# schusterbenjamin/Vision-Language-Pretraining-for-Bone-Tumor-Detection

Hardware: AMD Instinct MI355X
Metric: image-text pairs/sec (fwd+bwd) at bs=256/GPU, 1/2/4/8 MI355X (higher is better)
Workload: dtype bf16; 1 GPU; ResNet34+TinyBERT CLIP pretrain step (fwd+bwd+global-batch InfoNCE+AdamW); global_batch=256, per_gpu_batch=256, image_size=512, seq_len=40, parallelism=dp1

## Files before the change

include/vlp_hip.h:

```cpp
#ifndef VLP_HIP_H
#define VLP_HIP_H
#include <stdint.h>
#ifdef __cplusplus
extern "C" {
#endif

int vlp_abi_version(void);
int vlp_mfma_peak_probe(int blocks, int iters, float* out, void* stream);
int vlp_trace_marker(int end, void* stream);

int vlp_conv_fwd(int dtype, const void* x, const void* wp, void* y, int N, int H, int W, int C,
                 int Co, int KH, int KW, int S, int P, const float* in_scale,
                 const float* in_shift, double* stat_sum, double* stat_sumsq, int stat_rep,
                 void* stream);
int vlp_conv_fwd_act_ok(int dtype, int N, int H, int W, int C, int Co, int KH, int KW, int S, int P);
int vlp_conv_fwd_act(int dtype, const void* x, const void* wp, void* y, void* x_act, int N, int H, int W,
                     int C, int Co, int KH, int KW, int S, int P, const float* in_scale,
                     const float* in_shift, double* stat_sum, double* stat_sumsq, int stat_rep,
                     void* stream);
int vlp_conv_dgrad(int dtype, const void* dy, const void* wt, void* dx, int N, int H, int W, int C,
                   int Co, int KH, int KW, int S, int P, const void* addend, const void* y_bn,
                   const float* bn_scale, const float* bn_shift, const float* bn_mean,
                   const float* bn_invstd, double* stat1, double* stat2, int stat_rep,
                   void* stream);
int vlp_conv_dgrad_relu(int dtype, const void* dy, const void* wt, void* g, int N, int H, int W,
                        int C, int Co, int KH, int KW, int S, int P, const void* addend,
                        const void* relu_out, const uint8_t* relu_mask, const void* y,
                        const float* mean, const float* invstd, double* stat1, double* stat2,
                        int stat_rep, void* stream);
int vlp_conv_dgrad_act_ok(int dtype, int N, int H, int W, int C, int Co, int KH, int KW, int S, int P);
int vlp_conv_dgrad_bn_act(int dtype, const void* g_in, const void* y_in, const float* in_coef, void* dy_out,
                          const void* wt, void* dx, int N, int H, int W, int C, int Co, int KH, int KW,
                          int S, int P, const void* y_bn, const float* bn_scale, const float* bn_shift,
                          const float* bn_mean, const float* bn_invstd, double* stat1, double* stat2,
// ... 201 lines not shown
```

vision-language-pretraining-for-bone-tumor-detection_amd/csrc/bn_ops.hip:

```cpp
#include "common.h"

namespace vlp {

constexpr int kEwThreads = 256;

__device__ __forceinline__ uint8_t relu_bits8(const uint4& u) {
  const unsigned w[4] = {u.x, u.y, u.z, u.w};
  unsigned m = 0;
#pragma unroll
  for (int q = 0; q < 4; ++q) {
    const unsigned lo = w[q] & 0xffffu, hi = w[q] >> 16;
    m |= (unsigned)((lo & 0x8000u) == 0 && lo != 0) << (2 * q);
    m |= (unsigned)((hi & 0x8000u) == 0 && hi != 0) << (2 * q + 1);
  }
  return (uint8_t)m;
}

static inline int ew_blocks(size_t work, int per_block = kEwThreads, int cap = 8192) {
  size_t b = (work + per_block - 1) / per_block;
  if (b > (size_t)cap) b = cap;
  if (b < 1) b = 1;
  return (int)b;
}

__global__ void bn_finalize_kernel(int C, double count, const double* __restrict__ sum,
                                   const double* __restrict__ sumsq, const float* __restrict__ gamma,
                                   const float* __restrict__ beta, float eps, float momentum,
                                   float* running_mean, float* running_var, float* scale,
                                   float* shift, float* mean_out, float* invstd_out) {
  int c = blockIdx.x * blockDim.x + threadIdx.x;
  if (c >= C) return;
// ... 136 lines not shown
  const int c0 = (int)(tid % (unsigned)cpr) * E;
  float a[E], b[E], c[E], d[E];
#pragma unroll
  for (int j = 0; j < E; ++j) {
    a[j] = sc[c0 + j]; b[j] = sh[c0 + j];
    c[j] = scd ? scd[c0 + j] : 1.f;
    d[j] = scd ? shd[c0 + j] : 0.f;
    b[j] += d[j];
  }
  auto one = [&](unsigned i, const uint4& yv, const uint4& iv) __attribute__((always_inline)) {
    float u[E], v[E];
    Chunk<T>::unpack(yv, u);
    if constexpr (HAS_IDT) {
      Chunk<T>::unpack(iv, v);
#pragma unroll
      for (int j = 0; j < E; ++j) u[j] = fmaxf(fmaf(u[j], a[j], fmaf(v[j], c[j], b[j])), 0.f);
    } else {
#pragma unroll
      for (int j = 0; j < E; ++j) u[j] = fmaxf(fmaf(u[j], a[j], b[j]), 0.f);
    }
    const uint4 pk = Chunk<T>::pack(u);
    ew_st16<U, NT>(out + (size_t)i * E, pk);
    if constexpr (E == 8) {
      if (rmask) rmask[i] = relu_bits8(pk);
    }
  };
  unsigned i = tid;
  if constexpr (U > 1) {
    for (; i + (U - 1) * stride < nchunks; i += U * stride) {
      uint4 yv[U], iv[U];
#pragma unroll
// ... 45 lines not shown
      const unsigned i = i0 + 256u * k;
      if (i < nchunks) {
        yv[k] = NTL ? ntl16(y + (size_t)i * 8) : ldg16(y + (size_t)i * 8);
        if constexpr (HAS_IDT) iv[k] = NTL ? ntl16(idt + (size_t)i * 8) : ldg16(idt + (size_t)i * 8);
      }
    }
#pragma unroll
    for (int k = 0; k < U; ++k) {
      const unsigned i = i0 + 256u * k;
      if (i >= nchunks) continue;
      float u[8], v[8];
      Chunk<bf16>::unpack(yv[k], u);
      if constexpr (HAS_IDT) {
        Chunk<bf16>::unpack(iv[k], v);
#pragma unroll
        for (int j = 0; j < 8; ++j) u[j] = fmaxf(fmaf(u[j], a[j], fmaf(v[j], c[j], b[j])), 0.f);
      } else {
#pragma unroll
        for (int j = 0; j < 8; ++j) u[j] = fmaxf(fmaf(u[j], a[j], b[j]), 0.f);
      }
      const uint4 pk = Chunk<bf16>::pack(u);
      ew_st16<1, true>(out + (size_t)i * 8, pk);
      if (rmask) rmask[i] = relu_bits8(pk);
    }
  }
}

template <typename T>
__global__ void __launch_bounds__(256)
bn_bwd_reduce_kernel(int M, int C, const T* __restrict__ dout, const float* __restrict__ dbc,
                     int HW, const T* __restrict__ mask, const T* __restrict__ ya,
// ... 927 lines not shown
```

vision-language-pretraining-for-bone-tumor-detection_amd/csrc/common.h:

```cpp
#pragma once
#include <hip/hip_runtime.h>
#include <stdint.h>

namespace vlp {

typedef __bf16 bf16;
typedef float v4f __attribute__((ext_vector_type(4)));
typedef __bf16 v4bf __attribute__((ext_vector_type(4)));
typedef __bf16 v8bf __attribute__((ext_vector_type(8)));

enum { VLP_F32 = 0, VLP_BF16 = 1 };

template <typename T> struct Elem;
template <> struct Elem<bf16> {
  static constexpr int EPC = 8;
  static constexpr int BK = 64;
};
template <> struct Elem<float> {
  static constexpr int EPC = 4;
  static constexpr int BK = 32;
};

__device__ __forceinline__ float to_f(float x) { return x; }
__device__ __forceinline__ float to_f(bf16 x) { return (float)x; }
// ... 75 lines not shown
  return (t + ((n - t) >> f.s1)) >> f.s2;
}

__device__ __forceinline__ void bn_bwd_coef(float gamma, float istd, float mean, double sum_g, double sum_gx,
                                            float inv_count, float& k, float& b, float& c) {
  k = __fmul_rn(gamma, istd);
  const float mg = __fmul_rn((float)sum_g, inv_count), mgx = __fmul_rn((float)sum_gx, inv_count);
  const float t = __fmul_rn(__fmul_rn(k, istd), mgx);
  b = -t;
  c = __fadd_rn(-__fmul_rn(k, mg), __fmul_rn(t, mean));
}
__device__ __forceinline__ float bn_bwd_dy(float k, float b, float c, float g, float y) {
  return __fmaf_rn(k, g, __fmaf_rn(b, y, c));
}

__device__ __forceinline__ float warp_sum(float v) {
#pragma unroll
  for (int o = 32; o > 0; o >>= 1) v += __shfl_xor(v, o, 64);
  return v;
}
__device__ __forceinline__ float warp_max(float v) {
#pragma unroll
  for (int o = 32; o > 0; o >>= 1) v = fmaxf(v, __shfl_xor(v, o, 64));
  return v;
}

__device__ __forceinline__ float hash_uniform(uint64_t seed, uint64_t idx) {
  uint64_t z = seed + 0x9E3779B97F4A7C15ull * (idx + 1);
  z = (z ^ (z >> 30)) * 0xBF58476D1CE4E5B9ull;
  z = (z ^ (z >> 27)) * 0x94D049BB133111EBull;
// ... 11 lines not shown
```

vision-language-pretraining-for-bone-tumor-detection_amd/csrc/conv_ops.hip:

```cpp
#include "gemm.h"
#include "stem_geom.h"

namespace vlp {

struct ConvGeom {
  int N, H, W, C, Co, KH, KW, S, P, Ho, Wo;
  int M;
  int K;
  FastDiv fd_howo, fd_wo, fd_hw, fd_w, fd_c, fd_co, fd_kw;
};

static ConvGeom make_geom(int N, int H, int W, int C, int Co, int KH, int KW, int S, int P) {
  ConvGeom g;
  g.N = N; g.H = H; g.W = W; g.C = C; g.Co = Co; g.KH = KH; g.KW = KW; g.S = S; g.P = P;
  g.Ho = (H + 2 * P - KH) / S + 1;
  g.Wo = (W + 2 * P - KW) / S + 1;
  g.M = 0; g.K = 0;
  g.fd_howo = make_fastdiv(g.Ho * g.Wo);
  g.fd_wo = make_fastdiv(g.Wo);
  g.fd_hw = make_fastdiv(H * W);
  g.fd_w = make_fastdiv(W);
  g.fd_c = make_fastdiv(C);
  g.fd_co = make_fastdiv(Co);
  g.fd_kw = make_fastdiv(KW);
// ... 1128 lines not shown
constexpr int kRcRing = 5;
constexpr int kRcRingOff = kRcWeights;
constexpr int kRcAux = 0;
constexpr int kRcTail = kRcWeights + kRcRing * kRcSlot;
constexpr int kRcXtab = kRcTail + 2048;
constexpr int kRcLds = kRcXtab + 768;
static_assert(kRcLds <= 160 * 1024, "rows kernel LDS map");

#ifndef VLP_ACT_NT
#define VLP_ACT_NT 0
#endif
struct RowsXIn {
  const float* t0; const float* t1;
  const bf16* y;
  bf16* out;
};
template <class EP, int XF = 0>
__global__ void __launch_bounds__(512)
conv3x3_c64_rows_kernel(int N, int H, const bf16* __restrict__ x, const bf16* __restrict__ w, int flip,
                        EP ep, int M, RowsXIn xin) {
  constexpr int S = RowTrait<EP>::value ? 2 : 4;
  static_assert(XF != 1 || !RowTrait<EP>::value, "forward input transform with the direct epilogue only");
  static_assert(XF != 2 || RowTrait<EP>::value, "backward input transform with a row-chunk epilogue only");
  extern __shared__ __attribute__((aligned(16))) char smem[];
  char* wlds = smem;
  char* ring = smem + kRcRingOff;
  char* aux = smem + kRcAux;
  float* red = reinterpret_cast<float*>(RowTrait<EP>::value ? aux + 16384 : smem + kRcTail);
  const int tid = threadIdx.x, lane = tid & 63;
  const int wv = __builtin_amdgcn_readfirstlane((int)(tid >> 6));
  const int pq = wv & 3, ch = wv >> 2;
  const rsrc_t rx = buf_rsrc(x, (unsigned)((size_t)N * H * kRcW * 64 * 2));
  const rsrc_t rw = buf_rsrc(w, 64 * 576 * 2);
  const rsrc_t rz = null_rsrc(zero_page());

  for (int j = wv; j < 72; j += 8) {
    const int b = j >> 3, q = (j & 7) * 64 + lane;
// ... 46 lines not shown
    __syncthreads();
    v4f* rp = reinterpret_cast<v4f*>(red + tid * 16);
    rp[0] = rp[1] = rp[2] = rp[3] = v4f{0.f, 0.f, 0.f, 0.f};
  }
  constexpr int NCF = CoefTrait<EP>::value;
  float* cfl = reinterpret_cast<float*>(smem + kRcTail);
  if constexpr (NCF > 0) {
    for (int q = tid; q < NCF * 64; q += 512) cfl[q] = ep.coef(q >> 6)[q & 63];
    __syncthreads();
  }
  float* xtab = reinterpret_cast<float*>(smem + kRcXtab);
  if constexpr (XF == 1) {
    if (tid < 128) xtab[tid] = tid < 64 ? xin.t0[tid] : xin.t1[tid - 64];
    __syncthreads();
  }
  if constexpr (XF == 2) {
    if (tid < 192) xtab[tid] = xin.t0[tid];
    __syncthreads();
  }
  char* ybuf = aux + 16384 + 32768;
  static_assert(16384 + 32768 + kRcW * 128 <= kRcWeights, "y row buffer fits the filter area");
  const rsrc_t ry = XF == 2 ? buf_rsrc(xin.y, (unsigned)((size_t)N * H * kRcW * 64 * 2)) : rz;
  auto yload = [&](int n, int r) __attribute__((always_inline)) {
    const bool live = (unsigned)r < (unsigned)H;
    const rsrc_t rr = live ? ry : rz;
    const unsigned base = live ? (unsigned)(((size_t)n * H + r) * kRcW * 128) : 0u;
    int sd = lane;
    asm volatile("" : "+v"(sd));
#pragma unroll
    for (int jj = 0; jj < 2; ++jj) {
      const int j = wv * 2 + jj;
      int px, c;
      piece_src(j, sd, px, c);
      dma16(rr, base + (unsigned)(px * 128 + c * 16), ybuf + j * 1024);
    }
  };
  auto xrow = [&](int n, int r) __attribute__((always_inline)) {
// ... 5 lines not shown
      const int j = wv * 2 + jj, q = j * 64 + sd;
      int px, cc;
      piece_src(j, sd, px, cc);
      uint4* p = reinterpret_cast<uint4*>(piece_lds(slot, j) + sd * 16);
      float f[8];
      Chunk<bf16>::unpack(*p, f);
      if constexpr (XF == 2) {
        float yy[8];
        Chunk<bf16>::unpack(*reinterpret_cast<const uint4*>(ybuf + q * 16), yy);
#pragma unroll
        for (int j = 0; j < 8; ++j)
          f[j] = bn_bwd_dy(xtab[cc * 8 + j], xtab[64 + cc * 8 + j], xtab[128 + cc * 8 + j], f[j], yy[j]);
      } else {
        const v4f s0 = *reinterpret_cast<const v4f*>(xtab + cc * 8), s1 = *reinterpret_cast<const v4f*>(xtab + cc * 8 + 4);
        const v4f h0 = *reinterpret_cast<const v4f*>(xtab + 64 + cc * 8), h1 = *reinterpret_cast<const v4f*>(xtab + 68 + cc * 8);
#pragma unroll
        for (int j = 0; j < 4; ++j) {
          f[j] = fmaxf(fmaf(f[j], s0[j], h0[j]), 0.f);
          f[4 + j] = fmaxf(fmaf(f[4 + j], s1[j], h1[j]), 0.f);
        }
      }
      const uint4 v = Chunk<bf16>::pack(f);
      *p = v;
#if VLP_ACT_NT
      typedef unsigned v4u_nt __attribute__((ext_vector_type(4)));
      __builtin_nontemporal_store(v4u_nt{v.x, v.y, v.z, v.w},
                                  reinterpret_cast<v4u_nt*>(xin.out + (((size_t)n * H + r) * kRcW + px) * 64 + cc * 8));
#else
      stg16(xin.out + (((size_t)n * H + r) * kRcW + px) * 64 + cc * 8, v);
#endif
    }
  };

  for (int n = blockIdx.x; n < N; n += gridDim.x) {
    wait_vmcnt<0>();
    __syncthreads();
    if constexpr (XF == 2) {
      fetch(n, -1); fetch(n, 0); yload(n, 0);
    } else {
      fetch(n, -1); fetch(n, 0); fetch(n, 1); fetch(n, 2);
    }
    for (int i = 0; i < H; ++i) {
      if constexpr (XF == 2) {
        if (i == 0) {
          wait_vmcnt<0>();
          xrow(n, 0);
          yload(n, 1);
          fetch(n, 1);
          fetch(n, 2);
          wait_vmcnt<2>();
          xrow(n, 1);
        } else {
          wait_vmcnt<2 + S>();
          if (i + 1 < H) xrow(n, i + 1);
        }
        asm volatile("s_waitcnt lgkmcnt(0)" ::: "memory");
      } else {
        if (i == 0) wait_vmcnt<2>();
        else if (i == 1) wait_vmcnt<2 + S + (XF ? 4 : 0)>();
        else wait_vmcnt<2 + 2 * S + (XF ? 2 : 0)>();
        if constexpr (XF == 1) {
          if (i == 0) { xrow(n, 0); xrow(n, 1); }
          else if (i + 1 < H) xrow(n, i + 1);
          asm volatile("s_waitcnt lgkmcnt(0)" ::: "memory");
        }
      }
      raw_barrier();
      constexpr bool kRowEpi = RowTrait<EP>::value;
      if constexpr (!kRowEpi) fetch(n, i + 3);
      RowPre pre[2];
      if constexpr (kRowEpi) {
#pragma unroll
        for (int h2 = 0; h2 < 2; ++h2) ep.pre8((n * H + i) * kRcW + (tid >> 3) + 64 * h2, (tid & 7) * 8, pre[h2]);
        __builtin_amdgcn_sched_barrier(0);
        if constexpr (XF == 2) {
          yload(n, i + 2);
          __builtin_amdgcn_sched_barrier(0);
        }
        fetch(n, i + 3);
      }
      v4f acc[2][2];
#pragma unroll
      for (int a = 0; a < 2; ++a)
#pragma unroll
// ... 904 lines not shown
  if (!conv_chunks_ok(dtype, C, Co)) return (int)hipErrorInvalidValue;
  ConvGeom g = make_geom(N, H, W, C, Co, KH, KW, S, P);
  hipStream_t st = (hipStream_t)stream;
  if (dtype == VLP_BF16)
    return conv_fwd_t<bf16>(x, wp, y, g, in_scale, in_shift, stat_sum, stat_sumsq, stat_rep, st);
  return conv_fwd_t<float>(x, wp, y, g, in_scale, in_shift, stat_sum, stat_sumsq, stat_rep, st);
}

VLP_EXPORT int vlp_conv_fwd_act_ok(int dtype, int N, int H, int W, int C, int Co, int KH, int KW, int S,
                                  int P) {
  if (dtype != VLP_BF16 || N < 1) return 0;
  const ConvGeom g = make_geom(N, H, W, C, Co, KH, KW, S, P);
  return rows_c64_ok(g) ? 1 : 0;
}

VLP_EXPORT int vlp_conv_fwd_act(int dtype, const void* x, const void* wp, void* y, void* x_act, int N,
                                int H, int W, int C, int Co, int KH, int KW, int S, int P,
                                const float* in_scale, const float* in_shift, double* stat_sum,
                                double* stat_sumsq, int stat_rep, void* stream) {
  if (!vlp_conv_fwd_act_ok(dtype, N, H, W, C, Co, KH, KW, S, P) || !in_scale || !in_shift || !x_act ||
      !stat_sum || !stat_sumsq)
    return (int)hipErrorInvalidValue;
  ConvGeom g = make_geom(N, H, W, C, Co, KH, KW, S, P);
  g.M = g.N * g.Ho * g.Wo;
  g.K = g.KH * g.KW * g.C;
  EpiConvFwd<bf16> ep{stat_sum, stat_sumsq, stat_rep, (bf16*)y, g.Co};
  RowsXIn xin{};
  xin.t0 = in_scale;
  xin.t1 = in_shift;
  xin.out = (bf16*)x_act;
  return launch_rows_c64<EpiConvFwd<bf16>, 1>(g, x, wp, 0, ep, (hipStream_t)stream, xin);
}

static RowsXIn rows_bwd_xin(const void* y_in, const float* in_coef, void* dy_out) {
  RowsXIn xin{};
  xin.t0 = in_coef;
  xin.y = (const bf16*)y_in;
  xin.out = (bf16*)dy_out;
  return xin;
}

VLP_EXPORT int vlp_conv_dgrad_act_ok(int dtype, int N, int H, int W, int C, int Co, int KH, int KW, int S,
                                    int P) {
  return dtype == VLP_BF16 && N >= 1 && rows_c64_ok(make_geom(N, H, W, C, Co, KH, KW, S, P)) ? 1 : 0;
}

// ... 360 lines not shown
```

vision-language-pretraining-for-bone-tumor-detection_amd/vlp_amd/_lib.py:

```python
from __future__ import annotations

import ctypes
import os
import re
from typing import Dict, List

_HERE = os.path.dirname(os.path.abspath(__file__))
_PKG = os.path.dirname(_HERE)
_REPO = os.path.dirname(_PKG)
LIB_PATH = os.environ.get("VLP_HIP_LIB", os.path.join(_HERE, "libvlp_hip.so"))
HEADER_PATH = os.path.join(_REPO, "include", "vlp_hip.h")

F32, BF16 = 0, 1
ABI_VERSION = 3

_CTYPE = {
    "int": ctypes.c_int,
    "long long": ctypes.c_longlong,
    "unsigned long long": ctypes.c_ulonglong,
    "float": ctypes.c_float,
    "double": ctypes.c_double,
}


# ... 7 lines not shown
        ret, name, args = m.group(1), m.group(2), m.group(3).strip()
        parsed = []
        if args and args != "void":
            for a in args.split(","):
                a = " ".join(a.split())
                is_ptr = "*" in a
                a2 = a.replace("*", " ").replace("const ", "").strip()
                toks = a2.split()
                argname = toks[-1]
                tname = " ".join(toks[:-1])
                parsed.append(("ptr" if is_ptr else tname, argname))
        protos[name] = {"ret": ret, "args": parsed}
    return protos


_FAMILY_TIMED = {"vlp_conv_fwd", "vlp_conv_fwd_act", "vlp_conv_dgrad", "vlp_conv_dgrad_relu",
                 "vlp_conv_dgrad_bn_act", "vlp_conv_dgrad_relu_act", "vlp_conv_dgrad_relu_ds", "vlp_conv_dgrad_relu2", "vlp_conv_wgrad", "vlp_conv_wgrad_ws", "vlp_stem_fwd", "vlp_stem_wgrad", "vlp_stem_wgrad_ws",
                 "vlp_stem1_fwd", "vlp_stem1_wgrad_ws", "vlp_stem1_pool_fwd", "vlp_stem1_bwd_fused",
                 "vlp_linear_fwd", "vlp_linear_fwd_rs", "vlp_linear_dgrad", "vlp_linear_wgrad", "vlp_linear_wgrad_ws",
                 "vlp_nest_attn_fwd", "vlp_nest_attn_bwd"}


_QUERIES = {"vlp_linear_wgrad_ws_floats", "vlp_clip_loss_ws_floats", "vlp_stem1_bwd_fused_ws_floats",
            "vlp_stem1_fused_ok", "vlp_conv_fwd_act_ok", "vlp_conv_dgrad_act_ok"}


class HipError(RuntimeError):
    pass


class _Lib:
    def __init__(self, path: str = LIB_PATH):
        if not os.path.exists(path):
            raise ImportError(
                f"libvlp_hip.so not found at {path}: build it with "
                f"`python -c 'import __graft_entry__ as g; g.build()'` (no CPU fallback exists)")
        self._dll = ctypes.CDLL(path)
        self.protos = parse_header()
        self._fns = {}
# ... 60 lines not shown
```

vision-language-pretraining-for-bone-tumor-detection_amd/vlp_amd/ops.py:

```python
from __future__ import annotations

import torch

from . import ktimer
from ._lib import BF16, F32, lib, ptr, stream_of


def dcode(t: torch.Tensor) -> int:
    if t.dtype == torch.bfloat16:
        return BF16
    if t.dtype == torch.float32:
        return F32
    raise TypeError(f"unsupported storage dtype {t.dtype}")


def _s():
    return stream_of()


def conv_out_hw(H, W, KH, KW, S, P):
    return (H + 2 * P - KH) // S + 1, (W + 2 * P - KW) // S + 1


def _tile_auto(n):
# ... 17 lines not shown
        stat_sum = torch.zeros(Co, dtype=torch.float64, device=x.device)
        stat_sumsq = torch.zeros(Co, dtype=torch.float64, device=x.device)
    tk = ktimer.begin(f"conv_fwd[{'xf' if in_scale is not None else 'raw'}]{_tile_auto(Co)}",
                      2.0 * N * Ho * Wo * Co * C * KH * KW)
    lib().vlp_conv_fwd(dcode(x), ptr(x), ptr(wp), ptr(y), N, H, W, C, Co, KH, KW, S, P,
                       ptr(in_scale), ptr(in_shift), ptr(stat_sum), ptr(stat_sumsq), int(stat_rep), _s())
    ktimer.end(tk)
    return y


def conv_fwd_act_ok(x, Co, KH, KW, S, P):
    N, H, W, C = x.shape
    return bool(lib()._dll.vlp_conv_fwd_act_ok(dcode(x), N, H, W, C, Co, KH, KW, S, P))


def conv_fwd_act(x, wp, Co, KH, KW, S, P, in_scale, in_shift, x_act, stat_sum, stat_sumsq, stat_rep=1, out=None):
    N, H, W, C = x.shape
    Ho, Wo = conv_out_hw(H, W, KH, KW, S, P)
    y = out if out is not None else torch.empty((N, Ho, Wo, Co), dtype=x.dtype, device=x.device)
    tk = ktimer.begin("conv_fwd[act]/" + ("narrow" if C == 64 else "wide"), 2.0 * N * Ho * Wo * Co * C * KH * KW)
    lib().vlp_conv_fwd_act(dcode(x), ptr(x), ptr(wp), ptr(y), ptr(x_act), N, H, W, C, Co, KH, KW, S, P,
                           ptr(in_scale), ptr(in_shift), ptr(stat_sum), ptr(stat_sumsq), int(stat_rep), _s())
    ktimer.end(tk)
    return y


def conv_dgrad(dy, wt, H, W, C, KH, KW, S, P, addend=None, y_bn=None, bn=None, stat1=None,
               stat2=None, out=None, stat_rep=1):
    N, Ho, Wo, Co = dy.shape
    dx = out if out is not None else torch.empty((N, H, W, C), dtype=dy.dtype, device=dy.device)
    sc = sh = mu = ist = None
    if y_bn is not None:
        sc, sh, mu, ist = bn
    tk = ktimer.begin(f"conv_dgrad[{'bn' if y_bn is not None else 'add'}]{_tile_auto(C)}",
                      2.0 * N * Ho * Wo * Co * C * KH * KW)
    lib().vlp_conv_dgrad(dcode(dy), ptr(dy), ptr(wt), ptr(dx), N, H, W, C, Co, KH, KW, S, P,
                         ptr(addend), ptr(y_bn), ptr(sc), ptr(sh), ptr(mu), ptr(ist), ptr(stat1),
# ... 580 lines not shown
```

vision-language-pretraining-for-bone-tumor-detection_amd/vlp_amd/resnet34.py:

```python
from __future__ import annotations

from typing import List, Optional

import os

import torch
import torch.nn as nn

from . import ops
from .arena import ArenaModule

LAYERS = (3, 4, 6, 3)
WIDTHS = (64, 128, 256, 512)
BN_EPS = 1e-5
BN_MOMENTUM = 0.1
_USE_WG_STREAM = True
_WG_STREAMS = {}
STAT_REP = 64
_USE_STEM1 = os.environ.get("VLP_STEM1", "1") != "0"
_USE_STEM_FUSED = True
_USE_BWD_ACT = os.environ.get("VLP_BWD_ACT", "1") != "0"
_USE_DS_FOLD = os.environ.get("VLP_DS_FOLD", "1") != "0"
_USE_RELU2 = os.environ.get("VLP_RELU2", "1") != "0"
_USE_ACT_FUSED = True


def _side_stream(dev):
    s = _WG_STREAMS.get(dev)
    if s is None:
        s = _WG_STREAMS[dev] = torch.cuda.Stream(device=dev)
    return s


STAGES = ("stem", "layer1", "layer2", "layer3", "layer4")


def _stage_of(key: str) -> str:
    return key.split(".", 1)[0] if key.startswith("layer") else "stem"

# ... 91 lines not shown
                if b == 0 and (s != 1 or inpl != planes):
                    ds = nn.Sequential()
                    mk_conv(ds, "0", pre + ".downsample.0")
                    mk_bn(ds, "1", pre + ".downsample.1")
                    blk.downsample = ds
                layer.add_module(str(b), blk)
                inpl = planes
            setattr(self, f"layer{li + 1}", layer)
        self._blocks = []
        for li, n in enumerate(LAYERS):
            for b in range(n):
                pre = f"layer{li + 1}.{b}"
                self._blocks.append((pre, (pre + ".downsample.0") in self._convs))
        self.reset_parameters()
        self._ws = {}
        self._dbg = None
        self.u8_norm = (127.5, 73.9)

    @torch.no_grad()
    def reset_parameters(self, zero_init_last: bool = True):
        for c in self._convs.values():
            nn.init.kaiming_normal_(self.arena.view(c.key + ".weight"), mode="fan_out",
                                    nonlinearity="relu")
        for key in self._bns:
            self.arena.view(key + ".weight").fill_(1.0)
            self.arena.view(key + ".bias").zero_()
        if zero_init_last:
            for pre, _ in self._blocks:
                self.arena.view(pre + ".bn2.weight").zero_()

# ... 72 lines not shown
            desc = ops.pack_conv_batch(entries[0][1], entries)
            ws[key] = desc
        ops.pack_conv_batch_run(desc)
        ops.pack_stem(self.arena.view("conv1.weight"), ws["conv1.wp"])
        return ws

    def _bn_finalize(self, ws, key, count, training):
        bn = self._bns[key]
        gamma, beta = self.arena.view(key + ".weight"), self.arena.view(key + ".bias")
        sc, sh, mu, ist = self._coef(ws, key)
        h = bn.holder
        if training:
            s, ss = self._fstat(ws, key, full=True)
            ops.bn_finalize_rep(STAT_REP, count, s, ss, gamma, beta, BN_EPS, BN_MOMENTUM, h.running_mean,
                                h.running_var, sc, sh, mu, ist)
            h.num_batches_tracked.add_(1)
        else:
            ops.bn_eval_coeffs(gamma, beta, h.running_mean, h.running_var, BN_EPS, sc, sh)
        return sc, sh

    def run_forward(self, x: Optional[torch.Tensor], training: bool, x_u8: Optional[torch.Tensor] = None,
                    u8_norm=(127.5, 73.9)):
        ws = self.pack_weights()
        T = self.tdtype
        dev = self.arena.data.device
        src = x if x is not None else x_u8
        N, H, W = src.shape[0], src.shape[-2], src.shape[-1]
        ws["fstat"].zero_()
        g1 = ops.stem1_geom(H, W) if (x is None and _USE_STEM1) else None
        fused = g1 is not None and T == torch.bfloat16 and _USE_STEM_FUSED and ops.stem1_fused_ok(H, W)
        if fused:
            Ho, Wo, Hp, Wp1 = g1
            key = ("xs", N, H, W)
            xs = ws.get(key)
            if xs is None:
                xs = torch.empty(4, N, Hp, Wp1, dtype=T, device=dev)
                ws[key] = xs
            ops.stem1_prep_u8(x_u8.contiguous(), xs, u8_norm[0], u8_norm[1])
            if "conv1.wp1" not in ws:
                ws["conv1.wp1"] = torch.empty(64, 64, dtype=T, device=dev)
            ops.pack_stem1(self.arena.view("conv1.weight"), ws["conv1.wp1"])
            Hq, Wq = (Ho + 2 - 3) // 2 + 1, (Wo + 2 - 3) // 2 + 1
            yarg = torch.empty(N, Hq, Wq, 64, dtype=T, device=dev)
            idx = torch.empty(N, Hq, Wq, 64, dtype=torch.uint8, device=dev)
            s, ss = self._fstat(ws, "bn1", full=True) if training else (None, None)
            ops.stem1_pool_fwd(xs, ws["conv1.wp1"], self.arena.view("bn1.weight"), yarg, idx, N, H, W, s, ss,
                               STAT_REP)
            sc0, sh0 = self._bn_finalize(ws, "bn1", N * Ho * Wo, training)
            p = torch.empty(N, Hq, Wq, 64, dtype=T, device=dev)
            pm = torch.empty(p.numel() // 8, dtype=torch.uint8, device=dev) if training else None
            ops.bn_add_relu(yarg, sc0, sh0, None, None, None, p, relu_mask=pm)
            saved = {"N": N, "H": H, "W": W, "xs": xs, "training": training, "stem_fused": True,
                     "y0": None, "idx": idx, "yarg": yarg if training else None}
            return self._run_blocks(ws, T, dev, N, p, pm, saved, training)
        if g1 is not None:
            Ho, Wo, Hp, Wp1 = g1
            key = ("xs", N, H, W)
            xs = ws.get(key)
            if xs is None:
                xs = torch.empty(4, N, Hp, Wp1, dtype=T, device=dev)
                ws[key] = xs
            ops.stem1_prep_u8(x_u8.contiguous(), xs, u8_norm[0], u8_norm[1])
            if "conv1.wp1" not in ws:
                ws["conv1.wp1"] = torch.empty(64, 64, dtype=T, device=dev)
            ops.pack_stem1(self.arena.view("conv1.weight"), ws["conv1.wp1"])
            saved = {"N": N, "H": H, "W": W, "xs": xs, "training": training}
            y0 = torch.empty(N, Ho, Wo, 64, dtype=T, device=dev)
            s, ss = self._fstat(ws, "bn1", full=True)
            ops.stem1_fwd(xs, ws["conv1.wp1"], N, H, W, y0, s, ss, STAT_REP)
# ... 11 lines not shown
            saved = {"N": N, "H": H, "W": W, "xp": xp, "training": training}
            y0 = torch.empty(N, Ho, Wo, 64, dtype=T, device=dev)
            s, ss = self._fstat(ws, "bn1", full=True)
            ops.stem_fwd(xp, ws["conv1.wp"], N, H, W, y0, s, ss, STAT_REP)
        sc0, sh0 = self._bn_finalize(ws, "bn1", N * Ho * Wo, training)
        Hq, Wq = (Ho + 2 - 3) // 2 + 1, (Wo + 2 - 3) // 2 + 1
        p = torch.empty(N, Hq, Wq, 64, dtype=T, device=dev)
        idx = torch.empty(N, Hq, Wq, 64, dtype=torch.uint8, device=dev)
        yarg = torch.empty_like(p) if training else None
        bits = training and T == torch.bfloat16
        pm = torch.empty(p.numel() // 8, dtype=torch.uint8, device=dev) if bits else None
        ops.maxpool_fwd(y0, sc0, sh0, p, idx, yarg, relu_mask=pm)
        saved["y0"], saved["idx"], saved["yarg"] = y0, idx, yarg
        return self._run_blocks(ws, T, dev, N, p, pm, saved, training)

    def _run_blocks(self, ws, T, dev, N, p, pm, saved, training):
        bits = training and T == torch.bfloat16
        xmask = pm
        xcur = p
        blocks = []
        for pre, has_ds in self._blocks:
            blk, xcur, xmask = self._block_fwd(ws, T, dev, pre, has_ds, xcur, xmask, training, bits)
            blocks.append(blk)
        feat = torch.empty(N, 512, dtype=T, device=dev)
        ops.avgpool_fwd(xcur, feat)
        saved["blocks"] = blocks
        return feat, saved

    def _block_fwd(self, ws, T, dev, pre, has_ds, xcur, xmask, training, bits):
        c1, c2 = self._convs[pre + ".conv1"], self._convs[pre + ".conv2"]
        s, ss = self._fstat(ws, pre + ".bn1", full=True)
        y1 = ops.conv_fwd(xcur, ws[c1.key + ".wp"], c1.Co, 3, 3, c1.S, 1, stat_sum=s, stat_sumsq=ss,
                          stat_rep=STAT_REP)
        Mb = y1.numel() // y1.shape[-1]
        sc1, sh1 = self._bn_finalize(ws, pre + ".bn1", Mb, training)
        a1 = torch.empty_like(y1)
        s, ss = self._fstat(ws, pre + ".bn2", full=True)
        if _USE_ACT_FUSED and ops.conv_fwd_act_ok(y1, c2.Co, 3, 3, 1, 1):
            y2 = ops.conv_fwd_act(y1, ws[c2.key + ".wp"], c2.Co, 3, 3, 1, 1, sc1, sh1, a1, s, ss,
                                  stat_rep=STAT_REP)
        else:
            ops.bn_add_relu(y1, sc1, sh1, None, None, None, a1)
            y2 = ops.conv_fwd(a1, ws[c2.key + ".wp"], c2.Co, 3, 3, 1, 1, stat_sum=s, stat_sumsq=ss,
                              stat_rep=STAT_REP)
        sc2, sh2 = self._bn_finalize(ws, pre + ".bn2", Mb, training)
        yd = scd = shd = None
        if has_ds:
            cd = self._convs[pre + ".downsample.0"]
            s, ss = self._fstat(ws, pre + ".downsample.1", full=True)
            yd = ops.conv_fwd(xcur, ws[cd.key + ".wp"], cd.Co, 1, 1, cd.S, 0, stat_sum=s,
                              stat_sumsq=ss, stat_rep=STAT_REP)
            scd, shd = self._bn_finalize(ws, pre + ".downsample.1", Mb, training)
        out = torch.empty_like(y2)
        om = torch.empty(out.numel() // 8, dtype=torch.uint8, device=dev) if bits else None
        ops.bn_add_relu(y2, sc2, sh2, yd if has_ds else xcur, scd, shd, out, relu_mask=om)
        blk = {"x": xcur, "xmask": xmask, "y1": y1, "a1": a1, "y2": y2, "yd": yd, "out": out}
        return blk, out, om

    def stage_span(self, stage):
        return self.arena.span(self._stage_names[stage])

    def run_backward(self, saved, dfeat: torch.Tensor, on_stage_done=None):
        ws = self._workspace()
        T = self.tdtype
        dev = self.arena.data.device
        self._sw = _side_stream(dev) if (_USE_WG_STREAM and dev.type == "cuda") else None
        try:
            self._run_backward(saved, dfeat, ws, T, dev, on_stage_done)
        finally:
            if self._sw is not None:
                torch.cuda.current_stream(dev).wait_stream(self._sw)
            self._sw = None
# ... 7 lines not shown
        if self._sw is not None:
            self._sw.wait_stream(torch.cuda.current_stream(dev))
            with torch.cuda.stream(self._sw):
                cb(lo, hi - lo)
            return
        cb(lo, hi - lo)

    def run_block_range_forward(self, x: torch.Tensor, lo: int, hi: int, training: bool = True):
        ws = self.pack_weights()
        T = self.tdtype
        dev = self.arena.data.device
        if x.dtype != T or x.dim() != 4 or x.shape[-1] != self._convs[self._blocks[lo][0] + ".conv1"].C:
            raise ValueError(f"block range input must be NHWC {T} with the block's channel count, got "
                             f"{tuple(x.shape)} {x.dtype}")
        ws["fstat"].zero_()
        bits = training and T == torch.bfloat16
        xmask = None
        if bits:
            xmask = torch.empty(x.numel() // 8, dtype=torch.uint8, device=dev)
            C = x.shape[-1]
            one = torch.ones(C, dtype=torch.float32, device=dev)
            xr = torch.empty_like(x)
            ops.bn_add_relu(x, one, torch.zeros_like(one), None, None, None, xr, relu_mask=xmask)
        blocks = [None] * lo
        xcur = x
        for pre, has_ds in self._blocks[lo:hi]:
            blk, xcur, xmask = self._block_fwd(ws, T, dev, pre, has_ds, xcur, xmask, training, bits)
            blocks.append(blk)
        return xcur, {"blocks": blocks, "range": (lo, hi), "training": training}

    def run_block_range_backward(self, saved, dout: torch.Tensor):
        ws = self._workspace()
        dev = self.arena.data.device
        self._sw = _side_stream(dev) if (_USE_WG_STREAM and dev.type == "cuda") else None
        try:
            lo, hi = saved["range"]
            return self._run_backward(saved, None, ws, self.tdtype, dev, None, lo=lo, hi=hi,
                                      dout0=dout.to(self.tdtype).contiguous())
        finally:
            if self._sw is not None:
                torch.cuda.current_stream(dev).wait_stream(self._sw)
            self._sw = None

    def _run_backward(self, saved, dfeat, ws, T, dev, on_stage_done=None, lo=0, hi=None, dout0=None):
# ... 235 lines not shown
```

Baseline: 6527 image-text pairs/s.

## Fuse residual BN-add-ReLU into next block's conv1 input load

Adds a conv3x3 forward variant (XF==3) that takes the previous block's raw conv2 output and identity tensor and applies BN scale/shift, the residual add and ReLU while loading rows. It writes the activated tensor and its ReLU bitmask as side outputs. The stem's BN-ReLU is folded into the first conv the same way. This drops a separate elementwise bn_add_relu pass per eligible block, saving one full read and write of the activation. num_batches_tracked increments are also batched into a single foreach add. In exchange, the fused kernel has extra identity-row loads and more complex vmcnt scheduling, which may slow the conv mainloop.

```diff
diff --git a/include/vlp_hip.h b/include/vlp_hip.h
--- a/include/vlp_hip.h
+++ b/include/vlp_hip.h
@@ -18,6 +18,15 @@
                      int C, int Co, int KH, int KW, int S, int P, const float* in_scale,
                      const float* in_shift, double* stat_sum, double* stat_sumsq, int stat_rep,
                      void* stream);
+int vlp_conv_fwd_act_bits(int dtype, const void* x, const void* wp, void* y, void* x_act, uint8_t* x_bits,
+                          int N, int H, int W, int C, int Co, int KH, int KW, int S, int P,
+                          const float* in_scale, const float* in_shift, double* stat_sum,
+                          double* stat_sumsq, int stat_rep, void* stream);
+int vlp_conv_fwd_res_act_ok(int dtype, int N, int H, int W, int C, int Co, int KH, int KW, int S, int P);
+int vlp_conv_fwd_res_act(int dtype, const void* y_in, const void* idt, const void* wp, void* y, void* x_out,
+                         uint8_t* x_bits, int N, int H, int W, int C, int Co, int KH, int KW, int S, int P,
+                         const float* in_scale, const float* in_shift, double* stat_sum,
+                         double* stat_sumsq, int stat_rep, void* stream);
 int vlp_conv_dgrad(int dtype, const void* dy, const void* wt, void* dx, int N, int H, int W, int C,
                    int Co, int KH, int KW, int S, int P, const void* addend, const void* y_bn,
                    const float* bn_scale, const float* bn_shift, const float* bn_mean,
diff --git a/vision-language-pretraining-for-bone-tumor-detection_amd/csrc/bn_ops.hip b/vision-language-pretraining-for-bone-tumor-detection_amd/csrc/bn_ops.hip
--- a/vision-language-pretraining-for-bone-tumor-detection_amd/csrc/bn_ops.hip
+++ b/vision-language-pretraining-for-bone-tumor-detection_amd/csrc/bn_ops.hip
@@ -3,18 +3,6 @@
 namespace vlp {
 
 constexpr int kEwThreads = 256;
-
-__device__ __forceinline__ uint8_t relu_bits8(const uint4& u) {
-  const unsigned w[4] = {u.x, u.y, u.z, u.w};
-  unsigned m = 0;
-#pragma unroll
-  for (int q = 0; q < 4; ++q) {
-    const unsigned lo = w[q] & 0xffffu, hi = w[q] >> 16;
-    m |= (unsigned)((lo & 0x8000u) == 0 && lo != 0) << (2 * q);
-    m |= (unsigned)((hi & 0x8000u) == 0 && hi != 0) << (2 * q + 1);
-  }
-  return (uint8_t)m;
-}
 
 static inline int ew_blocks(size_t work, int per_block = kEwThreads, int cap = 8192) {
   size_t b = (work + per_block - 1) / per_block;
@@ -181,7 +169,7 @@
     if constexpr (HAS_IDT) {
       Chunk<T>::unpack(iv, v);
 #pragma unroll
-      for (int j = 0; j < E; ++j) u[j] = fmaxf(fmaf(u[j], a[j], fmaf(v[j], c[j], b[j])), 0.f);
+      for (int j = 0; j < E; ++j) u[j] = bn_res_relu(u[j], a[j], v[j], c[j], b[j]);
     } else {
 #pragma unroll
       for (int j = 0; j < E; ++j) u[j] = fmaxf(fmaf(u[j], a[j], b[j]), 0.f);
@@ -257,7 +245,7 @@
       if constexpr (HAS_IDT) {
         Chunk<bf16>::unpack(iv[k], v);
 #pragma unroll
-        for (int j = 0; j < 8; ++j) u[j] = fmaxf(fmaf(u[j], a[j], fmaf(v[j], c[j], b[j])), 0.f);
+        for (int j = 0; j < 8; ++j) u[j] = bn_res_relu(u[j], a[j], v[j], c[j], b[j]);
       } else {
 #pragma unroll
         for (int j = 0; j < 8; ++j) u[j] = fmaxf(fmaf(u[j], a[j], b[j]), 0.f);
diff --git a/vision-language-pretraining-for-bone-tumor-detection_amd/csrc/common.h b/vision-language-pretraining-for-bone-tumor-detection_amd/csrc/common.h
--- a/vision-language-pretraining-for-bone-tumor-detection_amd/csrc/common.h
+++ b/vision-language-pretraining-for-bone-tumor-detection_amd/csrc/common.h
@@ -113,6 +113,21 @@
   return __fmaf_rn(k, g, __fmaf_rn(b, y, c));
 }
 
+__device__ __forceinline__ float bn_res_relu(float y, float a, float idt, float c, float b) {
+  return fmaxf(fmaf(y, a, fmaf(idt, c, b)), 0.f);
+}
+__device__ __forceinline__ uint8_t relu_bits8(const uint4& u) {
+  const unsigned w[4] = {u.x, u.y, u.z, u.w};
+  unsigned m = 0;
+#pragma unroll
+  for (int q = 0; q < 4; ++q) {
+    const unsigned lo = w[q] & 0xffffu, hi = w[q] >> 16;
+    m |= (unsigned)((lo & 0x8000u) == 0 && lo != 0) << (2 * q);
+    m |= (unsigned)((hi & 0x8000u) == 0 && hi != 0) << (2 * q + 1);
+  }
+  return (uint8_t)m;
+}
+
 __device__ __forceinline__ float warp_sum(float v) {
 #pragma unroll
   for (int o = 32; o > 0; o >>= 1) v += __shfl_xor(v, o, 64);
diff --git a/vision-language-pretraining-for-bone-tumor-detection_amd/csrc/conv_ops.hip b/vision-language-pretraining-for-bone-tumor-detection_amd/csrc/conv_ops.hip
--- a/vision-language-pretraining-for-bone-tumor-detection_amd/csrc/conv_ops.hip
+++ b/vision-language-pretraining-for-bone-tumor-detection_amd/csrc/conv_ops.hip
@@ -1166,13 +1166,14 @@
   const float* t0; const float* t1;
   const bf16* y;
   bf16* out;
+  uint8_t* bits;
 };
 template <class EP, int XF = 0>
 __global__ void __launch_bounds__(512)
 conv3x3_c64_rows_kernel(int N, int H, const bf16* __restrict__ x, const bf16* __restrict__ w, int flip,
                         EP ep, int M, RowsXIn xin) {
   constexpr int S = RowTrait<EP>::value ? 2 : 4;
-  static_assert(XF != 1 || !RowTrait<EP>::value, "forward input transform with the direct epilogue only");
+  static_assert((XF != 1 && XF != 3) || !RowTrait<EP>::value, "forward input transform with the direct epilogue only");
   static_assert(XF != 2 || RowTrait<EP>::value, "backward input transform with a row-chunk epilogue only");
   extern __shared__ __attribute__((aligned(16))) char smem[];
   char* wlds = smem;
@@ -1249,13 +1250,17 @@
     if (tid < 128) xtab[tid] = tid < 64 ? xin.t0[tid] : xin.t1[tid - 64];
     __syncthreads();
   }
+  if constexpr (XF == 3) {
+    if (tid < 128) xtab[tid] = tid < 64 ? xin.t0[tid] : xin.t1[tid - 64] + 0.f;
+    __syncthreads();
+  }
   if constexpr (XF == 2) {
     if (tid < 192) xtab[tid] = xin.t0[tid];
     __syncthreads();
   }
   char* ybuf = aux + 16384 + 32768;
   static_assert(16384 + 32768 + kRcW * 128 <= kRcWeights, "y row buffer fits the filter area");
-  const rsrc_t ry = XF == 2 ? buf_rsrc(xin.y, (unsigned)((size_t)N * H * kRcW * 64 * 2)) : rz;
+  const rsrc_t ry = (XF == 2 || XF == 3) ? buf_rsrc(xin.y, (unsigned)((size_t)N * H * kRcW * 64 * 2)) : rz;
   auto yload = [&](int n, int r) __attribute__((always_inline)) {
     const bool live = (unsigned)r < (unsigned)H;
     const rsrc_t rr = live ? ry : rz;
@@ -1291,14 +1296,27 @@
       } else {
         const v4f s0 = *reinterpret_cast<const v4f*>(xtab + cc * 8), s1 = *reinterpret_cast<const v4f*>(xtab + cc * 8 + 4);
         const v4f h0 = *reinterpret_cast<const v4f*>(xtab + 64 + cc * 8), h1 = *reinterpret_cast<const v4f*>(xtab + 68 + cc * 8);
-#pragma unroll
-        for (int j = 0; j < 4; ++j) {
-          f[j] = fmaxf(fmaf(f[j], s0[j], h0[j]), 0.f);
-          f[4 + j] = fmaxf(fmaf(f[4 + j], s1[j], h1[j]), 0.f);
+        if constexpr (XF == 3) {
+          float id[8];
+          Chunk<bf16>::unpack(*reinterpret_cast<const uint4*>(ybuf + q * 16), id);
+#pragma unroll
+          for (int j = 0; j < 4; ++j) {
+            f[j] = bn_res_relu(f[j], s0[j], id[j], 1.f, h0[j]);
+            f[4 + j] = bn_res_relu(f[4 + j], s1[j], id[4 + j], 1.f, h1[j]);
+          }
+        } else {
+#pragma unroll
+          for (int j = 0; j < 4; ++j) {
+            f[j] = fmaxf(fmaf(f[j], s0[j], h0[j]), 0.f);
+            f[4 + j] = fmaxf(fmaf(f[4 + j], s1[j], h1[j]), 0.f);
+          }
         }
       }
       const uint4 v = Chunk<bf16>::pack(f);
       *p = v;
+      if constexpr (XF == 1 || XF == 3) {
+        if (xin.bits) xin.bits[(((size_t)n * H + r) * kRcW + px) * 8 + cc] = relu_bits8(v);
+      }
 #if VLP_ACT_NT
       typedef unsigned v4u_nt __attribute__((ext_vector_type(4)));
       __builtin_nontemporal_store(v4u_nt{v.x, v.y, v.z, v.w},
@@ -1314,6 +1332,10 @@
     __syncthreads();
     if constexpr (XF == 2) {
       fetch(n, -1); fetch(n, 0); yload(n, 0);
+    } else if constexpr (XF == 3) {
+      fetch(n, -1); fetch(n, 0); yload(n, 0);
+      __builtin_amdgcn_sched_barrier(0);
+      fetch(n, 1); fetch(n, 2);
     } else {
       fetch(n, -1); fetch(n, 0); fetch(n, 1); fetch(n, 2);
     }
@@ -1332,10 +1354,29 @@
           if (i + 1 < H) xrow(n, i + 1);
         }
         asm volatile("s_waitcnt lgkmcnt(0)" ::: "memory");
+      } else if constexpr (XF == 3) {
+        if (i == 0) {
+          wait_vmcnt<4>();
+          xrow(n, 0);
+          asm volatile("s_waitcnt lgkmcnt(0)" ::: "memory");
+          yload(n, 1);
+          wait_vmcnt<0>();
+          xrow(n, 1);
+        } else {
+          wait_vmcnt<2 + S>();
+          if (i + 1 < H) xrow(n, i + 1);
+        }
+        asm volatile("s_waitcnt lgkmcnt(0)" ::: "memory");
       } else {
+        const bool xb = XF == 1 && xin.bits != nullptr;
         if (i == 0) wait_vmcnt<2>();
-        else if (i == 1) wait_vmcnt<2 + S + (XF ? 4 : 0)>();
-        else wait_vmcnt<2 + 2 * S + (XF ? 2 : 0)>();
+        else if (i == 1) {
+          if (xb) wait_vmcnt<2 + S + 8>();
+          else wait_vmcnt<2 + S + (XF ? 4 : 0)>();
+        } else {
+          if (xb) wait_vmcnt<2 + 2 * S + 4>();
+          else wait_vmcnt<2 + 2 * S + (XF ? 2 : 0)>();
+        }
         if constexpr (XF == 1) {
           if (i == 0) { xrow(n, 0); xrow(n, 1); }
           else if (i + 1 < H) xrow(n, i + 1);
@@ -1344,7 +1385,13 @@
       }
       raw_barrier();
       constexpr bool kRowEpi = RowTrait<EP>::value;
-      if constexpr (!kRowEpi) fetch(n, i + 3);
+      if constexpr (!kRowEpi) {
+        if constexpr (XF == 3) {
+          yload(n, i + 2);
+          __builtin_amdgcn_sched_barrier(0);
+        }
+        fetch(n, i + 3);
+      }
       RowPre pre[2];
       if constexpr (kRowEpi) {
 #pragma unroll
@@ -2279,12 +2326,12 @@
   return rows_c64_ok(g) ? 1 : 0;
 }
 
-VLP_EXPORT int vlp_conv_fwd_act(int dtype, const void* x, const void* wp, void* y, void* x_act, int N,
-                                int H, int W, int C, int Co, int KH, int KW, int S, int P,
-                                const float* in_scale, const float* in_shift, double* stat_sum,
-                                double* stat_sumsq, int stat_rep, void* stream) {
-  if (!vlp_conv_fwd_act_ok(dtype, N, H, W, C, Co, KH, KW, S, P) || !in_scale || !in_shift || !x_act ||
-      !stat_sum || !stat_sumsq)
+VLP_EXPORT int vlp_conv_fwd_act_bits(int dtype, const void* x, const void* wp, void* y, void* x_act,
+                                     uint8_t* x_bits, int N, int H, int W, int C, int Co, int KH, int KW, int S,
+                                     int P, const float* in_scale, const float* in_shift, double* stat_sum,
+                                     double* stat_sumsq, int stat_rep, void* stream) {
+  if (!vlp_conv_fwd_act_ok(dtype, N, H, W, C, Co, KH, KW, S, P) || !x || !wp || !y || !in_scale || !in_shift ||
+      !x_act || !stat_sum || !stat_sumsq)
     return (int)hipErrorInvalidValue;
   ConvGeom g = make_geom(N, H, W, C, Co, KH, KW, S, P);
   g.M = g.N * g.Ho * g.Wo;
@@ -2294,7 +2341,41 @@
   xin.t0 = in_scale;
   xin.t1 = in_shift;
   xin.out = (bf16*)x_act;
+  xin.bits = x_bits;
   return launch_rows_c64<EpiConvFwd<bf16>, 1>(g, x, wp, 0, ep, (hipStream_t)stream, xin);
+}
+
+VLP_EXPORT int vlp_conv_fwd_act(int dtype, const void* x, const void* wp, void* y, void* x_act, int N,
+                                int H, int W, int C, int Co, int KH, int KW, int S, int P,
+                                const float* in_scale, const float* in_shift, double* stat_sum,
+                                double* stat_sumsq, int stat_rep, void* stream) {
+  return vlp_conv_fwd_act_bits(dtype, x, wp, y, x_act, nullptr, N, H, W, C, Co, KH, KW, S, P, in_scale, in_shift,
+                               stat_sum, stat_sumsq, stat_rep, stream);
+}
+
+VLP_EXPORT int vlp_conv_fwd_res_act_ok(int dtype, int N, int H, int W, int C, int Co, int KH, int KW, int S,
+                                      int P) {
+  return vlp_conv_fwd_act_ok(dtype, N, H, W, C, Co, KH, KW, S, P);
+}
+
+VLP_EXPORT int vlp_conv_fwd_res_act(int dtype, const void* y_in, const void* idt, const void* wp, void* y,
+                                    void* x_out, uint8_t* x_bits, int N, int H, int W, int C, int Co, int KH,
+                                    int KW, int S, int P, const float* in_scale, const float* in_shift,
+                                    double* stat_sum, double* stat_sumsq, int stat_rep, void* stream) {
+  if (!vlp_conv_fwd_res_act_ok(dtype, N, H, W, C, Co, KH, KW, S, P) || !y_in || !idt || !wp || !y || !x_out ||
+      !in_scale || !in_shift || !stat_sum || !stat_sumsq)
+    return (int)hipErrorInvalidValue;
+  ConvGeom g = make_geom(N, H, W, C, Co, KH, KW, S, P);
+  g.M = g.N * g.Ho * g.Wo;
+  g.K = g.KH * g.KW * g.C;
+  EpiConvFwd<bf16> ep{stat_sum, stat_sumsq, stat_rep, (bf16*)y, g.Co};
+  RowsXIn xin{};
+  xin.t0 = in_scale;
+  xin.t1 = in_shift;
+  xin.y = (const bf16*)idt;
+  xin.out = (bf16*)x_out;
+  xin.bits = x_bits;
+  return launch_rows_c64<EpiConvFwd<bf16>, 3>(g, y_in, wp, 0, ep, (hipStream_t)stream, xin);
 }
 
 static RowsXIn rows_bwd_xin(const void* y_in, const float* in_coef, void* dy_out) {
diff --git a/vision-language-pretraining-for-bone-tumor-detection_amd/vlp_amd/_lib.py b/vision-language-pretraining-for-bone-tumor-detection_amd/vlp_amd/_lib.py
--- a/vision-language-pretraining-for-bone-tumor-detection_amd/vlp_amd/_lib.py
+++ b/vision-language-pretraining-for-bone-tumor-detection_amd/vlp_amd/_lib.py
@@ -45,7 +45,7 @@
     return protos
 
 
-_FAMILY_TIMED = {"vlp_conv_fwd", "vlp_conv_fwd_act", "vlp_conv_dgrad", "vlp_conv_dgrad_relu",
+_FAMILY_TIMED = {"vlp_conv_fwd", "vlp_conv_fwd_act", "vlp_conv_fwd_act_bits", "vlp_conv_fwd_res_act", "vlp_conv_dgrad", "vlp_conv_dgrad_relu",
                  "vlp_conv_dgrad_bn_act", "vlp_conv_dgrad_relu_act", "vlp_conv_dgrad_relu_ds", "vlp_conv_dgrad_relu2", "vlp_conv_wgrad", "vlp_conv_wgrad_ws", "vlp_stem_fwd", "vlp_stem_wgrad", "vlp_stem_wgrad_ws",
                  "vlp_stem1_fwd", "vlp_stem1_wgrad_ws", "vlp_stem1_pool_fwd", "vlp_stem1_bwd_fused",
                  "vlp_linear_fwd", "vlp_linear_fwd_rs", "vlp_linear_dgrad", "vlp_linear_wgrad", "vlp_linear_wgrad_ws",
@@ -53,7 +53,7 @@
 
 
 _QUERIES = {"vlp_linear_wgrad_ws_floats", "vlp_clip_loss_ws_floats", "vlp_stem1_bwd_fused_ws_floats",
-            "vlp_stem1_fused_ok", "vlp_conv_fwd_act_ok", "vlp_conv_dgrad_act_ok"}
+            "vlp_stem1_fused_ok", "vlp_conv_fwd_act_ok", "vlp_conv_fwd_res_act_ok", "vlp_conv_dgrad_act_ok"}
 
 
 class HipError(RuntimeError):
diff --git a/vision-language-pretraining-for-bone-tumor-detection_amd/vlp_amd/ops.py b/vision-language-pretraining-for-bone-tumor-detection_amd/vlp_amd/ops.py
--- a/vision-language-pretraining-for-bone-tumor-detection_amd/vlp_amd/ops.py
+++ b/vision-language-pretraining-for-bone-tumor-detection_amd/vlp_amd/ops.py
@@ -55,13 +55,44 @@
     return bool(lib()._dll.vlp_conv_fwd_act_ok(dcode(x), N, H, W, C, Co, KH, KW, S, P))
 
 
-def conv_fwd_act(x, wp, Co, KH, KW, S, P, in_scale, in_shift, x_act, stat_sum, stat_sumsq, stat_rep=1, out=None):
+def conv_fwd_act(x, wp, Co, KH, KW, S, P, in_scale, in_shift, x_act, stat_sum, stat_sumsq, stat_rep=1, out=None,
+                 x_bits=None):
     N, H, W, C = x.shape
     Ho, Wo = conv_out_hw(H, W, KH, KW, S, P)
     y = out if out is not None else torch.empty((N, Ho, Wo, Co), dtype=x.dtype, device=x.device)
-    tk = ktimer.begin("conv_fwd[act]/" + ("narrow" if C == 64 else "wide"), 2.0 * N * Ho * Wo * Co * C * KH * KW)
+    tile = "narrow" if C == 64 else "wide"
+    if x_bits is not None:
+        tk = ktimer.begin("conv_fwd[act,bits]/" + tile, 2.0 * N * Ho * Wo * Co * C * KH * KW)
+        lib().vlp_conv_fwd_act_bits(dcode(x), ptr(x), ptr(wp), ptr(y), ptr(x_act), ptr(x_bits), N, H, W, C, Co,
+                                    KH, KW, S, P, ptr(in_scale), ptr(in_shift), ptr(stat_sum), ptr(stat_sumsq),
+                                    int(stat_rep), _s())
+        ktimer.end(tk)
+        return y
+    tk = ktimer.begin("conv_fwd[act]/" + tile, 2.0 * N * Ho * Wo * Co * C * KH * KW)
     lib().vlp_conv_fwd_act(dcode(x), ptr(x), ptr(wp), ptr(y), ptr(x_act), N, H, W, C, Co, KH, KW, S, P,
                            ptr(in_scale), ptr(in_shift), ptr(stat_sum), ptr(stat_sumsq), int(stat_rep), _s())
+    ktimer.end(tk)
+    return y
+
+
+def conv_fwd_res_act_ok(x, Co, KH, KW, S, P):
+    N, H, W, C = x.shape
+    return bool(lib()._dll.vlp_conv_fwd_res_act_ok(dcode(x), N, H, W, C, Co, KH, KW, S, P))
+
+
+def conv_fwd_res_act(y_in, idt, wp, Co, KH, KW, S, P, in_scale, in_shift, x_out, x_bits, stat_sum, stat_sumsq,
+                     stat_rep=1, out=None):
+    N, H, W, C = y_in.shape
+    if idt.shape != y_in.shape or x_out.shape != y_in.shape or idt.dtype != y_in.dtype or x_out.dtype != y_in.dtype \
+            or (x_bits is not None and x_bits.numel() * 8 != y_in.numel()):
+        raise ValueError("conv_fwd_res_act: identity, output and bits must match the input's shape")
+    Ho, Wo = conv_out_hw(H, W, KH, KW, S, P)
+    y = out if out is not None else torch.empty((N, Ho, Wo, Co), dtype=y_in.dtype, device=y_in.device)
+    tk = ktimer.begin("conv_fwd[res,act]/" + ("narrow" if C == 64 else "wide"),
+                      2.0 * N * Ho * Wo * Co * C * KH * KW)
+    lib().vlp_conv_fwd_res_act(dcode(y_in), ptr(y_in), ptr(idt), ptr(wp), ptr(y), ptr(x_out), ptr(x_bits), N, H, W,
+                               C, Co, KH, KW, S, P, ptr(in_scale), ptr(in_shift), ptr(stat_sum), ptr(stat_sumsq),
+                               int(stat_rep), _s())
     ktimer.end(tk)
     return y
 
diff --git a/vision-language-pretraining-for-bone-tumor-detection_amd/vlp_amd/resnet34.py b/vision-language-pretraining-for-bone-tumor-detection_amd/vlp_amd/resnet34.py
--- a/vision-language-pretraining-for-bone-tumor-detection_amd/vlp_amd/resnet34.py
+++ b/vision-language-pretraining-for-bone-tumor-detection_amd/vlp_amd/resnet34.py
@@ -23,6 +23,7 @@
 _USE_DS_FOLD = os.environ.get("VLP_DS_FOLD", "1") != "0"
 _USE_RELU2 = os.environ.get("VLP_RELU2", "1") != "0"
 _USE_ACT_FUSED = True
+_USE_RES_FUSED = os.environ.get("VLP_RES_FUSED", "1") != "0"
 
 
 def _side_stream(dev):
@@ -144,6 +145,7 @@
                 self._blocks.append((pre, (pre + ".downsample.0") in self._convs))
         self.reset_parameters()
         self._ws = {}
+        self._nbt_pending = []
         self._dbg = None
         self.u8_norm = (127.5, 73.9)
 
@@ -246,7 +248,7 @@
             s, ss = self._fstat(ws, key, full=True)
             ops.bn_finalize_rep(STAT_REP, count, s, ss, gamma, beta, BN_EPS, BN_MOMENTUM, h.running_mean,
                                 h.running_var, sc, sh, mu, ist)
-            h.num_batches_tracked.add_(1)
+            self._nbt_pending.append(h.num_batches_tracked)
         else:
             ops.bn_eval_coeffs(gamma, beta, h.running_mean, h.running_var, BN_EPS, sc, sh)
         return sc, sh
@@ -259,6 +261,7 @@
         src = x if x is not None else x_u8
         N, H, W = src.shape[0], src.shape[-2], src.shape[-1]
         ws["fstat"].zero_()
+        self._nbt_pending = []
         g1 = ops.stem1_geom(H, W) if (x is None and _USE_STEM1) else None
         fused = g1 is not None and T == torch.bfloat16 and _USE_STEM_FUSED and ops.stem1_fused_ok(H, W)
         if fused:
@@ -281,10 +284,15 @@
             sc0, sh0 = self._bn_finalize(ws, "bn1", N * Ho * Wo, training)
             p = torch.empty(N, Hq, Wq, 64, dtype=T, device=dev)
             pm = torch.empty(p.numel() // 8, dtype=torch.uint8, device=dev) if training else None
-            ops.bn_add_relu(yarg, sc0, sh0, None, None, None, p, relu_mask=pm)
+            pend = None
+            c1 = self._convs[self._blocks[0][0] + ".conv1"]
+            if _USE_RES_FUSED and ops.conv_fwd_act_ok(yarg, c1.Co, 3, 3, c1.S, 1):
+                pend = (yarg, sc0, sh0, None)
+            else:
+                ops.bn_add_relu(yarg, sc0, sh0, None, None, None, p, relu_mask=pm)
             saved = {"N": N, "H": H, "W": W, "xs": xs, "training": training, "stem_fused": True,
                      "y0": None, "idx": idx, "yarg": yarg if training else None}
-            return self._run_blocks(ws, T, dev, N, p, pm, saved, training)
+            return self._run_blocks(ws, T, dev, N, p, pm, saved, training, pend)
         if g1 is not None:
             Ho, Wo, Hp, Wp1 = g1
             key = ("xs", N, H, W)
@@ -326,24 +334,45 @@
         saved["y0"], saved["idx"], saved["yarg"] = y0, idx, yarg
         return self._run_blocks(ws, T, dev, N, p, pm, saved, training)
 
-    def _run_blocks(self, ws, T, dev, N, p, pm, saved, training):
+    def _run_blocks(self, ws, T, dev, N, p, pm, saved, training, pend=None):
         bits = training and T == torch.bfloat16
-        xmask = pm
-        xcur = p
-        blocks = []
-        for pre, has_ds in self._blocks:
-            blk, xcur, xmask = self._block_fwd(ws, T, dev, pre, has_ds, xcur, xmask, training, bits)
-            blocks.append(blk)
+        blocks, xcur, _ = self._blocks_fwd(ws, T, dev, 0, len(self._blocks), p, pm, training, bits, pend)
         feat = torch.empty(N, 512, dtype=T, device=dev)
         ops.avgpool_fwd(xcur, feat)
         saved["blocks"] = blocks
         return feat, saved
 
-    def _block_fwd(self, ws, T, dev, pre, has_ds, xcur, xmask, training, bits):
+    def _blocks_fwd(self, ws, T, dev, lo, hi, xcur, xmask, training, bits, pend=None):
+        blocks = []
+        for bi in range(lo, hi):
+            pre, has_ds = self._blocks[bi]
+            nxt = None
+            if _USE_RES_FUSED and bi + 1 < hi and not has_ds and not self._blocks[bi + 1][1]:
+                nxt = self._convs[self._blocks[bi + 1][0] + ".conv1"]
+            blk, xcur, xmask, pend = self._block_fwd(ws, T, dev, pre, has_ds, xcur, xmask, training, bits, pend, nxt)
+            blocks.append(blk)
+        self._nbt_flush()
+        return blocks, xcur, xmask
+
+    def _nbt_flush(self):
+        if self._nbt_pending:
+            torch._foreach_add_(self._nbt_pending, 1)
+            self._nbt_pending = []
+
+    def _block_fwd(self, ws, T, dev, pre, has_ds, xcur, xmask, training, bits, pend=None, nxt=None):
         c1, c2 = self._convs[pre + ".conv1"], self._convs[pre + ".conv2"]
         s, ss = self._fstat(ws, pre + ".bn1", full=True)
-        y1 = ops.conv_fwd(xcur, ws[c1.key + ".wp"], c1.Co, 3, 3, c1.S, 1, stat_sum=s, stat_sumsq=ss,
-                          stat_rep=STAT_REP)
+        if pend is not None:
+            py, psc, psh, pid = pend
+            if pid is None:
+                y1 = ops.conv_fwd_act(py, ws[c1.key + ".wp"], c1.Co, 3, 3, c1.S, 1, psc, psh, xcur, s, ss,
+                                      stat_rep=STAT_REP, x_bits=xmask)
+            else:
+                y1 = ops.conv_fwd_res_act(py, pid, ws[c1.key + ".wp"], c1.Co, 3, 3, c1.S, 1, psc, psh, xcur, xmask,
+                                          s, ss, stat_rep=STAT_REP)
+        else:
+            y1 = ops.conv_fwd(xcur, ws[c1.key + ".wp"], c1.Co, 3, 3, c1.S, 1, stat_sum=s, stat_sumsq=ss,
+                              stat_rep=STAT_REP)
         Mb = y1.numel() // y1.shape[-1]
         sc1, sh1 = self._bn_finalize(ws, pre + ".bn1", Mb, training)
         a1 = torch.empty_like(y1)
@@ -365,9 +394,13 @@
             scd, shd = self._bn_finalize(ws, pre + ".downsample.1", Mb, training)
         out = torch.empty_like(y2)
         om = torch.empty(out.numel() // 8, dtype=torch.uint8, device=dev) if bits else None
-        ops.bn_add_relu(y2, sc2, sh2, yd if has_ds else xcur, scd, shd, out, relu_mask=om)
+        pend = None
+        if nxt is not None and not has_ds and ops.conv_fwd_res_act_ok(y2, nxt.Co, nxt.KH, nxt.KW, nxt.S, nxt.P):
+            pend = (y2, sc2, sh2, xcur)
+        else:
+            ops.bn_add_relu(y2, sc2, sh2, yd if has_ds else xcur, scd, shd, out, relu_mask=om)
         blk = {"x": xcur, "xmask": xmask, "y1": y1, "a1": a1, "y2": y2, "yd": yd, "out": out}
-        return blk, out, om
+        return blk, out, om, pend
 
     def stage_span(self, stage):
         return self.arena.span(self._stage_names[stage])
@@ -405,6 +438,7 @@
             raise ValueError(f"block range input must be NHWC {T} with the block's channel count, got "
                              f"{tuple(x.shape)} {x.dtype}")
         ws["fstat"].zero_()
+        self._nbt_pending = []
         bits = training and T == torch.bfloat16
         xmask = None
         if bits:
@@ -413,12 +447,8 @@
             one = torch.ones(C, dtype=torch.float32, device=dev)
             xr = torch.empty_like(x)
             ops.bn_add_relu(x, one, torch.zeros_like(one), None, None, None, xr, relu_mask=xmask)
-        blocks = [None] * lo
-        xcur = x
-        for pre, has_ds in self._blocks[lo:hi]:
-            blk, xcur, xmask = self._block_fwd(ws, T, dev, pre, has_ds, xcur, xmask, training, bits)
-            blocks.append(blk)
-        return xcur, {"blocks": blocks, "range": (lo, hi), "training": training}
+        done, xcur, xmask = self._blocks_fwd(ws, T, dev, lo, hi, x, xmask, training, bits)
+        return xcur, {"blocks": [None] * lo + done, "range": (lo, hi), "training": training}
 
     def run_block_range_backward(self, saved, dout: torch.Tensor):
         ws = self._workspace()
```

Measured after the change: 6587 image-text pairs/s, median of 6. No clear change (+0.9%).
